# asharakeh/bayes-od-rc

Hardware: AMD Instinct MI355X
Metric: images/sec at N=10 MC samples, 512x512; per-anchor covariance latency (higher is better)
Workload: dtype bf16; 1 GPU; ResNet-50 RetinaNet + covar head, N=10 MC-dropout, 512x512, full BayesOD pipeline (forward+posterior+soft-NMS+cluster-fuse); global_batch=512, mc_samples=10, anchors=49104, parallelism=one GPU (no exchange; N > 1: image-sharded, one RCCL gather/step), visible_gpus=1, gpu_max_hw_queues=4

## Files before the change

### bayes-od-rc_amd/csrc/engine.hip

```cpp
#include "../../include/bayesod.h"
#include "kernels.h"
#include "jpeg_entropy.h"
#include "png_inflate.h"

#include <algorithm>
#include <array>
#include <atomic>
#include <chrono>
#include <cmath>
#include <condition_variable>
#include <deque>
#include <functional>
#include <mutex>
#include <thread>
#include <tuple>
#include <type_traits>
#include <cstdarg>
#include <cstdio>
#include <cstring>
#include <map>
#include <memory>
#include <string>
#include <system_error>
#include <vector>
#include <dlfcn.h>

namespace {

constexpr float BN_EPS = 1e-3f;

thread_local std::string g_create_error;

struct HostTensor { std::vector<int64_t> shape; std::vector<float> data; };

struct Plane {
    char* d = nullptr;
    int64_t base = 0;
    int64_t bstride = 0;
    int h = 0, w = 0, C = 0, pitch = 0;
};

struct PackedConv { char* w = nullptr; float* bias = nullptr; int cout = 0, cout_pad = 0, taps = 0, kw = 0, cin = 0; };

struct Op {
    enum Kind { STEM, POOL, CONV, KEEP } kind;
    ConvArgs conv;
    bool is_head3x3 = false;
    double flops = 0;
    std::string name;
    std::string wname[3], bnname[3];
    bool same_geom = false;
    int flavour = 0;
    int head[3] = {-1, -1, -1};
    bool hx_pyramid = false;
// ... 207 lines not shown
    int32_t* energy_list = nullptr; float* energy_term = nullptr;

    int sh = 0, sw = 0, ph = 0, pw = 0;
    int ch[6] = {0}, cw[6] = {0};
    int nlev = 0; int lh[8] = {0}, lw[8] = {0};
    int64_t lvl_off[8] = {0};
    int64_t lvl_p0[8] = {0};
    int64_t Ppad = 0; int P = 0, A = 0;

    std::map<std::string, HostTensor> host_w;
    std::map<std::string, PackedConv> packed;
    float* stem_w = nullptr; float* stem_b = nullptr;
    bool weights_ready = false, anchors_ready = false, forward_done = false, posterior_done = false,
         nms_done = false, cluster_done = false;

    float* d_images = nullptr;
    float* splitk_partial = nullptr; size_t splitk_elems = 0;
    uint8_t* d_frames_u8 = nullptr; size_t frames_u8_cap = 0;
    float* d_images_b[2] = {nullptr, nullptr}; uint8_t* d_u8_b[2] = {nullptr, nullptr}; size_t u8_cap_b[2] = {0, 0};
    hipStream_t copy = nullptr;
    hipEvent_t ev_img_ready[2] = {nullptr, nullptr}, ev_img_free[2] = {nullptr, nullptr};
    bool img_ready_pending[2] = {false, false}, img_free_pending[2] = {false, false};
    int cur_img_buf = -1;
    struct RaggedTable { std::vector<char> host; char* dev = nullptr; };
    RaggedTable rag_sync, rag_b[2];
    RaggedTable aug_sync, aug_b[2];
    JpegSlot jpeg_slot[3];
    PngSlot png_slot[3];
    CorruptSpec corrupt_pending;
    CorruptSlot corrupt_slot[3];
    hipEvent_t ev_tab[2] = {nullptr, nullptr};
    const float* kscale_src[2] = {nullptr, nullptr};
    float* kscale_cur[2] = {nullptr, nullptr}; int kscale_i = 0;
    const float* kscale_now = nullptr;
    char* stem_out = nullptr;
    int es = 2;
    bool split = false;
    char* pyr_hx = nullptr;
    int pyr_fmt = 1;
    int plan_mx = 0;
    int mx = 0;
    Plane pyramid;
    char* head_act[3][2] = {{nullptr}};
    char* head_act_t[3][4] = {{nullptr}};
    float* raw[3] = {nullptr};
    float* agg[3] = {nullptr};
    bool agg_plan = false;
    bool plan_fused_out = false, plan_xreuse = false, plan_xreuse0 = false;
    bool raw_valid = false, agg_valid = false;
    bool plan_sparse = false;
    bool plan_halo = false;
    SparseTailArgs sparse{};
    int plan_tail_rows = 0;
    bool agg_sparse = false;
    float* stat_acc[3] = {nullptr};
    int stat_k = 0;
    hipEvent_t ev_stat = nullptr;
    float* d_mirror = nullptr;
    int mirror_sym = -1, mirror_bad_level = 0;
    bool keep_ready = false;
    uint64_t keep_seed = 0; uint32_t keep_first = 0;
    uint64_t last_seed = 0; uint32_t last_first_image = 0;
    int32_t last_sample_base = 0;
    std::map<std::string, RowEnt*> tables;
    struct XrTable { RowEnt* rows = nullptr; int2* ext = nullptr; int m = 0; };
    std::map<std::string, XrTable> xr_tables;
    std::vector<Op> ops;
    const float* cur_images = nullptr;

    float* d_anchors = nullptr;
    PostBuffers pb{};
    float* nms_scores = nullptr; int32_t* nms_begin = nullptr;
    int32_t* nms_sel_s[2] = {nullptr, nullptr}; int32_t* nms_nsel_s[2] = {nullptr, nullptr};
    float* out_scores_s[2] = {nullptr, nullptr}; float* out_means_s[2] = {nullptr, nullptr};
    float* out_covs_s[2] = {nullptr, nullptr}; float* out_counts_s[2] = {nullptr, nullptr};
    int32_t* nms_sel = nullptr; int32_t* nms_nsel = nullptr;
    float* out_scores = nullptr; float* out_means = nullptr; float* out_covs = nullptr; float* out_counts = nullptr;
    int slot = 0;
    float* parts = nullptr;
    float* out_parts_s[2] = {nullptr, nullptr}; float* out_parts = nullptr;
    std::vector<char> parts_ok, det_parts_ok[2];
    bool parts_staged[2] = {false, false};
    bool class_parts = false;
    float* ent = nullptr; float* stat_ent = nullptr; int stat_ent_k = 0;
    float* cparts = nullptr;
    float* out_cparts_s[2] = {nullptr, nullptr}; float* out_cparts = nullptr;
    std::vector<char> cparts_ok, det_cparts_ok[2];
    bool cparts_staged[2] = {false, false};
    hipStream_t side = nullptr;
    int overlap_mode = 0;
    int ov_front_slots = 0, ov_slots = 0;
    hipStream_t full = nullptr, front = nullptr, back = nullptr;
    hipEvent_t ev_front_done[2] = {nullptr, nullptr}, ev_l0_done[2] = {nullptr, nullptr}, ev_join = nullptr;
    bool l0_pending[2] = {false, false};
    bool ov_dirty = false;
    char* pyr_d[2] = {nullptr, nullptr};
    int fwd_parity = 0, pyr_last = 0;
    int first_head_op = 0;
    bool in_overlap_call = false;
    int n_cu = 256;
    hipEvent_t ev_posterior = nullptr; hipEvent_t ev_done[2] = {nullptr, nullptr};
    int dev_op_lo = 0, dev_op_hi = 1 << 30;
    hipStream_t done_stream[2] = {nullptr, nullptr};
    bool side_pending[2] = {false, false};
    char* host_stage[2] = {nullptr, nullptr};
    float* rec_send = nullptr; float* rec_recv = nullptr; size_t rec_recv_elems = 0;
// ... 17 lines not shown
        va_list ap; va_start(ap, fmt); vsnprintf(buf, sizeof buf, fmt, ap); va_end(ap);
        err = buf;
        return s;
    }
    template <typename T> bod_status dalloc(T** p, size_t n_elems, bool zero = true) {
        void* q = nullptr;
        const size_t bytes = std::max<size_t>(n_elems * sizeof(T), 256);
        hipError_t e = hipMalloc(&q, bytes);
        if (e != hipSuccess) return fail(BOD_ERR_OOM, "hipMalloc(%zu) failed: %s", bytes, hipGetErrorString(e));
        if (zero) {
            e = hipMemsetAsync(q, 0, bytes, stream);
            if (e != hipSuccess) return fail(BOD_ERR_HIP, "hipMemset: %s", hipGetErrorString(e));
        }
        allocs.push_back(q);
        alloc_bytes[q] = bytes;
        device_bytes += (int64_t)bytes;
        *p = reinterpret_cast<T*>(q);
        return BOD_OK;
    }
};

#define HIPCHK(h, expr)                                                                         \
    do {                                                                                        \
        hipError_t _e = (expr);                                                                 \
        if (_e != hipSuccess)                                                                   \
            return (h)->fail(BOD_ERR_HIP, "%s failed: %s (%s:%d)", #expr, hipGetErrorString(_e), \
                             __FILE__, __LINE__);                                               \
    } while (0)
#define BODCHK(expr) do { bod_status _s = (expr); if (_s != BOD_OK) return _s; } while (0)

namespace {

const char* kHeadPrefix[3] = {"pyramid_classification", "pyramid_regression", "pyramid_cov"};
const int kHeadConvs[3] = {4, 3, 4};

void cu_slot_mask(int lo, int hi, uint32_t mask[8]) {
    for (int w = 0; w < 8; ++w) mask[w] = 0u;
    for (int slot = lo; slot < hi; ++slot)
        for (int xcd = 0; xcd < 8; ++xcd) { const int bit = slot * 8 + xcd; mask[bit >> 5] |= 1u << (bit & 31); }
}

int same_pad_before(int in, int k, int s) {
    const int out = (in + s - 1) / s;
    const int total = std::max((out - 1) * s + k - in, 0);
    return total / 2;
}

bod_status new_plane(bod_context* h, Plane* p, int B, int hh, int ww, int C) {
    p->h = hh; p->w = ww; p->C = C; p->pitch = ww + 2; p->base = 0;
    p->bstride = (int64_t)(hh + 2) * (ww + 2);
    return h->dalloc(&p->d, (size_t)B * p->bstride * C * h->es);
}

bod_status make_table(bod_context* h, const std::string& key, int B, const Plane& in, const Plane& out,
                      int stride, int org_y, int org_x, const Plane* res, const RowEnt** tbl) {
    auto it = h->tables.find(key);
    if (it != h->tables.end()) { *tbl = it->second; return BOD_OK; }
    std::vector<RowEnt> rows((size_t)B * out.h * out.w);
    size_t r = 0;
    for (int b = 0; b < B; ++b)
        for (int y = 0; y < out.h; ++y)
            for (int x = 0; x < out.w; ++x) {
                RowEnt e{};
                e.in_off = (int32_t)(in.base + b * in.bstride + (int64_t)(y * stride + org_y) * in.pitch + (x * stride + org_x));
                e.in_pitch = in.pitch;
                e.out_off = (int32_t)(out.base + b * out.bstride + (int64_t)(y + 1) * out.pitch + (x + 1));
                if (res) {
                    int ry = y, rx = x;
                    if (res->h != out.h || res->w != out.w) {
                        ry = std::min((int)std::floor((y + 0.5) * ((double)res->h / out.h)), res->h - 1);
                        rx = std::min((int)std::floor((x + 0.5) * ((double)res->w / out.w)), res->w - 1);
                    }
                    e.res_off = (int32_t)(res->base + b * res->bstride + (int64_t)(ry + 1) * res->pitch + (rx + 1));
                }
                rows[r++] = e;
            }
    RowEnt* d = nullptr;
    BODCHK(h->dalloc(&d, rows.size(), false));
    HIPCHK(h, hipMemcpyAsync(d, rows.data(), rows.size() * sizeof(RowEnt), hipMemcpyHostToDevice, h->stream));
    HIPCHK(h, hipStreamSynchronize(h->stream));
    h->tables[key] = d;
    *tbl = d;
    return BOD_OK;
}

const HostTensor* find_w(bod_context* h, const std::string& name, int kind) {
    auto it = h->host_w.find(name + "/" + std::to_string(kind));
    return it == h->host_w.end() ? nullptr : &it->second;
}

bod_status pack_conv(bod_context* h, const std::string& name, const std::string& bn, int cout_pad_to,
                     PackedConv* out, int hx = 0) {
    const std::string ckey = hx == 2 ? name + ":h4" : hx ? name + ":hx" : name;
    auto it = h->packed.find(ckey);
    if (it != h->packed.end()) { *out = it->second; return BOD_OK; }
    const HostTensor* k = find_w(h, name, 0);
    if (!k || k->shape.size() != 4) return h->fail(BOD_ERR_NOT_READY, "missing conv kernel '%s'", name.c_str());
    const int kh = (int)k->shape[0], kw = (int)k->shape[1], cin = (int)k->shape[2], cout = (int)k->shape[3];
    const HostTensor* b = find_w(h, name, 1);
    std::vector<double> scale(cout, 1.0), shift(cout, 0.0);
    for (int o = 0; o < cout; ++o) shift[o] = b ? (double)b->data[o] : 0.0;
    if (!bn.empty()) {
        const HostTensor *g = find_w(h, bn, 2), *be = find_w(h, bn, 3), *mu = find_w(h, bn, 4), *var = find_w(h, bn, 5);
        if (!g || !be || !mu || !var) return h->fail(BOD_ERR_NOT_READY, "missing batch-norm '%s'", bn.c_str());
        for (int o = 0; o < cout; ++o) {
            const double s = (double)g->data[o] / std::sqrt((double)var->data[o] + (double)BN_EPS);
            scale[o] = s;
            shift[o] = (shift[o] - (double)mu->data[o]) * s + (double)be->data[o];
        }
    }
    PackedConv pc;
    pc.cout = cout; pc.taps = kh * kw; pc.kw = kw; pc.cin = cin;
    pc.cout_pad = ((cout + cout_pad_to - 1) / cout_pad_to) * cout_pad_to;
    const size_t nw = (size_t)pc.cout_pad * pc.taps * cin;
    const bool as_f32 = h->es == 4 && !h->split;
    std::vector<uint16_t> w(as_f32 ? 0 : nw * (h->split ? 2 : 1), 0);
    std::vector<float> w32(as_f32 ? nw : 0, 0.f);
    std::vector<float> bias(pc.cout_pad, 0.f);
    for (int o = 0; o < cout; ++o) {
        bias[o] = (float)shift[o];
        for (int t = 0; t < pc.taps; ++t)
            for (int c = 0; c < cin; ++c) {
                const double v = (double)k->data[((size_t)t * cin + c) * cout + o] * scale[o];
                const size_t idx = ((size_t)o * pc.taps + t) * cin + c;
                if (h->split) {
                    const float f = (float)v;
                    const uint16_t hi = f2bf(f);
                    const size_t slot = ((size_t)o * pc.taps + t) * 2 * cin + (size_t)(c >> 5) * 64 + (c & 31);
                    w[slot] = hi; w[slot + 32] = f2bf(f - bf2f(hi));
// ... 5 lines not shown
        if (!h->split || cin % 64 != 0) return h->fail(BOD_ERR_INVALID_ARG, "hx weights need the (hi, lo) data path and cin %% 64 == 0");
        std::vector<float> row(cin);
        uint8_t* wb = reinterpret_cast<uint8_t*>(w.data());
        for (int o = 0; o < cout; ++o)
            for (int t = 0; t < pc.taps; ++t) {
                for (int c = 0; c < cin; ++c) row[c] = (float)((double)k->data[((size_t)t * cin + c) * cout + o] * scale[o]);
                if (hx == 2) {
                    if (cin != 256) return h->fail(BOD_ERR_INVALID_ARG, "h4 weights: 256 input channels");
                    pack_h4_row(row.data(), cin, wb + ((size_t)o * pc.taps + t) * cin * 4, true);
                } else pack_hx_row(row.data(), cin, wb + ((size_t)o * pc.taps + t) * cin * 4, true);
            }
    }
    size_t w_extra = 0;
    if (hx == 2) {
        if (pc.cout_pad != 256) return h->fail(BOD_ERR_INVALID_ARG, "h4 weights: one 256-cout tile");
        w_extra = (size_t)pc.taps * 2 * 2048;
        w.resize(w.size() + w_extra / 2, 0);
        uint8_t* wb = reinterpret_cast<uint8_t*>(w.data());
        uint8_t* sc = wb + nw * h->es;
        for (int t = 0; t < pc.taps; ++t)
            for (int x = 0; x < 2; ++x)
                for (int o = 0; o < 256; ++o)
                    std::memcpy(sc + ((size_t)(t * 2 + x) * 256 + o) * 8, wb + ((size_t)o * pc.taps + t) * cin * 4 + 768 + 8 * x, 8);
    }
    BODCHK(h->dalloc(&pc.w, nw * h->es + w_extra, false));
    BODCHK(h->dalloc(&pc.bias, bias.size(), false));
    HIPCHK(h, hipMemcpyAsync(pc.w, as_f32 ? (const void*)w32.data() : (const void*)w.data(), nw * h->es + w_extra,
                             hipMemcpyHostToDevice, h->stream));
    HIPCHK(h, hipMemcpyAsync(pc.bias, bias.data(), bias.size() * 4, hipMemcpyHostToDevice, h->stream));
    HIPCHK(h, hipStreamSynchronize(h->stream));
    h->packed[ckey] = pc;
    *out = pc;
    return BOD_OK;
}

ConvArgs base_args(const PackedConv& pc, const RowEnt* rows, int M, int in_cstride, int out_cstride) {
    ConvArgs a{};
    a.rows = rows; a.M = M; a.taps = pc.taps; a.KW = pc.kw; a.cin = pc.cin;
    a.in_cstride = in_cstride; a.cout_pad = pc.cout_pad; a.cout_valid = pc.cout;
    a.out_cstride = out_cstride; a.res_cstride = out_cstride; a.groups = 1;
    a.fan_count = 1; a.fan_stride = 0;
    return a;
}

void to_split_args(ConvArgs* a) {
    a->split = 1;
    a->cin *= 2; a->in_cstride *= 2; a->res_cstride *= 2;
    if (!(a->flags & CONV_OUT_F32)) a->out_cstride *= 2;
    for (int g = 0; g < 3; ++g) a->g[g].in_coff *= 2;
}

bod_status add_conv(bod_context* h, const std::string& name, const std::string& bn, const Plane& in,
                    const Plane& out, int stride, bool same, bool relu, const Plane* res,
                    char* out_relu = nullptr) {
    PackedConv pc;
    BODCHK(pack_conv(h, name, bn, 64, &pc));
    if (pc.cin != in.C || pc.cout != out.C)
        return h->fail(BOD_ERR_INVALID_ARG, "conv '%s': weight shape [%d->%d] does not match planes [%d->%d]",
                       name.c_str(), pc.cin, pc.cout, in.C, out.C);
    const int kh = pc.taps / pc.kw;
    int oy = 1, ox = 1;
    if (same) { oy = 1 - same_pad_before(in.h, kh, stride); ox = 1 - same_pad_before(in.w, pc.kw, stride); }
    char key[256];
    snprintf(key, sizeof key, "pp:%lld,%lld,%d:%lld,%lld,%d,%d,%d:%d:%d:%d:%lld,%lld,%d,%d,%d", (long long)in.base,
             (long long)in.bstride, in.pitch, (long long)out.base, (long long)out.bstride, out.pitch, out.h, out.w,
             stride, oy, ox, res ? (long long)res->base : -1LL, res ? (long long)res->bstride : 0LL,
             res ? res->pitch : 0, res ? res->h : 0, res ? res->w : 0);
    const RowEnt* tbl = nullptr;
    const int B = h->cfg.batch;
    BODCHK(make_table(h, key, B, in, out, stride, oy, ox, res, &tbl));
    Op op; op.kind = Op::CONV;
    op.conv = base_args(pc, tbl, B * out.h * out.w, in.C, out.C);
    op.conv.g[0] = ConvGroup{in.d, pc.w, pc.bias, out.d, res ? res->d : nullptr, out_relu, 0, 0, nullptr, nullptr, nullptr, 0, 0};
    op.conv.flags = relu ? CONV_RELU : 0;
    op.flops = 2.0 * op.conv.M * pc.cout * pc.taps * pc.cin;
    op.name = name; op.wname[0] = name; op.bnname[0] = bn;
    op.same_geom = stride == 1 && same && pc.taps == 9 && pc.kw == 3 && in.base == out.base && in.bstride == out.bstride && in.pitch == out.pitch &&
                   in.h == out.h && in.w == out.w;
    if (stride == 1 && same && pc.taps == 9 && pc.kw == 3 && in.h == out.h && in.w == out.w) { op.conv.plane_h = out.h; op.conv.plane_w = out.w; }
    static const bool splitk_on = [] { const char* e = getenv("BOD_CONV_SPLITK"); return !e || atoi(e) != 0; }();
    if (splitk_on && (h->es == 2 || h->split)) {
        const long tiles = (long)((op.conv.M + 127) / 128) * (pc.cout_pad % 128 == 0 ? pc.cout_pad / 128 : pc.cout_pad / 64);
        const int chunks = pc.cin * (h->split ? 2 : 1) / 64;
        int S = 1;
        while (tiles * S < 256 && S * 2 <= 16 && chunks % (S * 2) == 0 && (long)pc.taps * (chunks / (S * 2)) >= 4) S *= 2;
        if (S > 1) {
            op.conv.ksplit = S;
            h->splitk_elems = std::max(h->splitk_elems, (size_t)S * op.conv.M * pc.cout_pad);
        }
    }
    static const bool plane_xr_on = [] { const char* e = getenv("BOD_PLANE_XREUSE"); return !e || atoi(e) != 0; }();
    static const bool xr_on = [] { const char* e = getenv("BOD_CONV_XREUSE"); return !e || atoi(e) != 0; }();
    if (plane_xr_on && xr_on && (h->es == 2 || h->split) && !h->cfg.training && op.conv.ksplit <= 1 && stride == 1 && same && pc.taps == 9 && pc.kw == 3 &&
        pc.cin == 256 && pc.cout == 256 && pc.cout_pad == 256 && !res && !out_relu && in.h == out.h && in.w == out.w) {
        ConvArgs probe = op.conv;
        if (conv_igemm_uses_full_cout_tile(probe)) {
            const std::string xkey = std::string(key) + ":xr";
            auto it = h->xr_tables.find(xkey);
            if (it == h->xr_tables.end()) {
                std::vector<RowEnt> rows((size_t)op.conv.M), tiled;
                std::vector<ExtRow> ext;
                HIPCHK(h, hipMemcpy(rows.data(), tbl, rows.size() * sizeof(RowEnt), hipMemcpyDeviceToHost));
                if (!xr_tile_rows(rows, tiled, ext)) return h->fail(BOD_ERR_INVALID_ARG, "row-reuse tiling of '%s': extended rows out of order", name.c_str());
                bod_context::XrTable t;
                t.m = (int)tiled.size();
                BODCHK(h->dalloc(&t.rows, tiled.size(), false));
                BODCHK(h->dalloc(&t.ext, ext.size(), false));
                HIPCHK(h, hipMemcpy(t.rows, tiled.data(), tiled.size() * sizeof(RowEnt), hipMemcpyHostToDevice));
                HIPCHK(h, hipMemcpy(t.ext, ext.data(), ext.size() * sizeof(int2), hipMemcpyHostToDevice));
                it = h->xr_tables.emplace(xkey, t).first;
            }
            op.conv.rows = it->second.rows; op.conv.ext = it->second.ext; op.conv.M = it->second.m; op.conv.xreuse = 2;
        }
    }
    h->ops.push_back(op);
    return BOD_OK;
}

bod_status build_geometry(bod_context* h) {
    const bod_config& c = h->cfg;
    const int H = c.image_h, W = c.image_w;
    if (H < 64 || W < 64) return h->fail(BOD_ERR_INVALID_ARG, "image size %dx%d too small", H, W);
    h->sh = (H - 7) / 2 + 1; h->sw = (W - 7) / 2 + 1;
    h->ph = (h->sh + 2 - 3) / 2 + 1; h->pw = (h->sw + 4 - 3) / 2 + 1;
    h->ch[2] = h->ph; h->cw[2] = h->pw;
    for (int s = 3; s <= 5; ++s) { h->ch[s] = (h->ch[s - 1] - 1) / 2 + 1; h->cw[s] = (h->cw[s - 1] - 1) / 2 + 1; }
    if (c.min_level != 3 || c.max_level != 7)
        return h->fail(BOD_ERR_INVALID_ARG, "only pyramid levels 3..7 are supported (got %d..%d)", c.min_level, c.max_level);
    h->nlev = 5;
    h->lh[0] = h->ch[3]; h->lw[0] = h->cw[3];
    h->lh[1] = h->ch[4]; h->lw[1] = h->cw[4];
    h->lh[2] = h->ch[5]; h->lw[2] = h->cw[5];
    h->lh[3] = (h->lh[2] + 1) / 2; h->lw[3] = (h->lw[2] + 1) / 2;
    h->lh[4] = (h->lh[3] + 1) / 2; h->lw[4] = (h->lw[3] + 1) / 2;
    int64_t pp = 0; int p = 0;
    for (int l = 0; l < 5; ++l) {
        const int stride = 1 << (l + 3);
        const int ah = (H + stride - 1) / stride, aw = (W + stride - 1) / stride;
        if (ah != h->lh[l] || aw != h->lw[l])
            return h->fail(BOD_ERR_INVALID_ARG,
                           "pyramid level p%d is %dx%d but the anchor grid is %dx%d for a %dx%d image "
                           "(the reference's tf.concat of head outputs with anchors would mismatch too)",
                           l + 3, h->lh[l], h->lw[l], ah, aw, H, W);
        h->lvl_off[l] = pp; h->lvl_p0[l] = p;
        pp += (int64_t)(h->lh[l] + 2) * (h->lw[l] + 2);
        p += h->lh[l] * h->lw[l];
    }
    h->Ppad = pp; h->P = p; h->A = p * c.anchors_per_location;
    return BOD_OK;
}

Plane level_view(bod_context* h, int l) {
    Plane v = h->pyramid;
    v.base = h->lvl_off[l]; v.h = h->lh[l]; v.w = h->lw[l]; v.pitch = h->lw[l] + 2;
    return v;
}

bod_status ensure_raw(bod_context* h) {
    const bod_config& c = h->cfg;
    const int out_ch[3] = {c.anchors_per_location * c.num_classes, c.anchors_per_location * 4, c.anchors_per_location * 10};
    for (int hd = 0; hd < 3; ++hd) {
        if ((hd == 2 && !c.has_covar_head) || h->raw[hd]) continue;
        BODCHK(h->dalloc(&h->raw[hd], (size_t)c.batch * c.mc_samples * h->P * out_ch[hd]));
    }
    for (Op& o : h->ops)
// ... 4 lines not shown
}

bod_status train_init(bod_context* h);
bod_status train_forward_only(bod_context* h, const float* dev, uint64_t seed, uint32_t first_image_id);
const uint32_t* train_dyn_rng(bod_context* h);
void train_destroy(bod_context* h);
void val_destroy(bod_context* h);

bod_status ensure_stat(bod_context* h) {
    if (h->stat_acc[0]) return BOD_OK;
    const bod_config& c = h->cfg;
    const size_t BA = (size_t)c.batch * h->A;
    BODCHK(h->dalloc(&h->stat_acc[0], BA * c.num_classes));
    BODCHK(h->dalloc(&h->stat_acc[1], BA * 16));
    if (c.has_covar_head) BODCHK(h->dalloc(&h->stat_acc[2], BA * 10));
    if (c.covariance_parts & BOD_PARTS_CLASS) BODCHK(h->dalloc(&h->stat_ent, BA));
    return BOD_OK;
}

bod_status build_plan(bod_context* h) {
    const bod_config& c = h->cfg;
    const int B = c.batch, N = c.mc_samples;
    const bool train_mode = c.training != 0;
    h->ops.clear();
    {
        const HostTensor* k = find_w(h, "conv1", 0);
        if (!k || k->shape.size() != 4 || k->shape[0] != 7 || k->shape[2] != 3 || k->shape[3] != 64)
            return h->fail(BOD_ERR_NOT_READY, "missing / malformed stem kernel 'conv1' [7,7,3,64]");
        const HostTensor* b = find_w(h, "conv1", 1);
        const HostTensor *g = find_w(h, "bn_conv1", 2), *be = find_w(h, "bn_conv1", 3), *mu = find_w(h, "bn_conv1", 4), *var = find_w(h, "bn_conv1", 5);
        if (!g || !be || !mu || !var) return h->fail(BOD_ERR_NOT_READY, "missing batch-norm 'bn_conv1'");
        std::vector<float> w(7 * 7 * 3 * 64), bias(64);
        for (int o = 0; o < 64; ++o) {
            const double s = (double)g->data[o] / std::sqrt((double)var->data[o] + (double)BN_EPS);
            bias[o] = (float)((((b ? (double)b->data[o] : 0.0) - (double)mu->data[o]) * s) + (double)be->data[o]);
            for (int t = 0; t < 147; ++t) w[(size_t)t * 64 + o] = (float)((double)k->data[(size_t)t * 64 + o] * s);
        }
        BODCHK(h->dalloc(&h->stem_w, w.size(), false));
        BODCHK(h->dalloc(&h->stem_b, bias.size(), false));
        HIPCHK(h, hipMemcpyAsync(h->stem_w, w.data(), w.size() * 4, hipMemcpyHostToDevice, h->stream));
        HIPCHK(h, hipMemcpyAsync(h->stem_b, bias.data(), bias.size() * 4, hipMemcpyHostToDevice, h->stream));
        HIPCHK(h, hipStreamSynchronize(h->stream));
        BODCHK(h->dalloc(&h->stem_out, (size_t)B * h->sh * h->sw * 64 * h->es));
        Op s; s.kind = Op::STEM; s.name = "conv1(stem)"; s.flops = 2.0 * B * h->sh * h->sw * 64.0 * 147.0; h->ops.push_back(s);
        Op p; p.kind = Op::POOL; p.name = "pool1"; h->ops.push_back(p);
    }
    Plane x;
    BODCHK(new_plane(h, &x, B, h->ph, h->pw, 64));
    Plane pool_out = x;
    h->ops[1].conv.g[0].out = pool_out.d;
    const char* blocks[6] = {"", "", "abc", "abcd", c.backbone_depth == 101 ? "abcdefghijklmnopqrstuvw" : "abcdef", "abc"};
    const int f1s[6] = {0, 0, 64, 128, 256, 512};
    Plane taps[6];
    for (int st = 2; st <= 5; ++st) {
        const int f1 = f1s[st], f3 = f1 * 4, hh = h->ch[st], ww = h->cw[st];
        const int first_stride = st == 2 ? 1 : 2;
        Plane t1, t2, sc, oa, ob;
        BODCHK(new_plane(h, &t1, B, hh, ww, f1));
        BODCHK(new_plane(h, &t2, B, hh, ww, f1));
        BODCHK(new_plane(h, &sc, B, hh, ww, f3));
        BODCHK(new_plane(h, &oa, B, hh, ww, f3));
        BODCHK(new_plane(h, &ob, B, hh, ww, f3));
        bool use_a = true;
        int chain_stages = 0;
        if (const char* e = getenv("BOD_CHAIN_FUSION")) chain_stages = atoi(e);
        bool chain_ok = h->es == 2 && !h->split && !train_mode && ((st == 2 && chain_stages >= 1) || (st == 3 && chain_stages >= 3));
        Plane t1alt;
        if (chain_ok) BODCHK(new_plane(h, &t1alt, B, hh, ww, f1));
        bool t1_ready = false;
        bool pw_t1_ready = false;
        for (const char* bl = blocks[st]; *bl; ++bl) {
            char cb[64], bb[64];
            snprintf(cb, sizeof cb, "res%d%c_branch", st, *bl);
            snprintf(bb, sizeof bb, "bn%d%c_branch", st, *bl);
            const std::string c_(cb), b_(bb);
            if (chain_ok) {
                Plane& out = use_a ? oa : ob;
                const bool first = *bl == 'a';
                if (!t1_ready) BODCHK(add_conv(h, c_ + "2a", b_ + "2a", x, t1, first ? first_stride : 1, false, true, nullptr));
                if (first) BODCHK(add_conv(h, c_ + "1", b_ + "1", x, sc, first_stride, false, false, nullptr));
                BODCHK(add_conv(h, c_ + "2b", b_ + "2b", t1, t2, 1, true, true, nullptr));
                Op& op2b = h->ops.back();
                const Plane& shortcut = first ? sc : x;
                const bool can = op2b.conv.ksplit <= 1 && !conv_igemm_uses_big_tile(op2b.conv) && op2b.conv.cout_pad == f1 && (f1 == 64 || f1 == 128);
                if (!can) {
                    BODCHK(add_conv(h, c_ + "2c", b_ + "2c", t2, out, 1, false, true, &shortcut));
                    t1_ready = false;
                } else {
                    PackedConv p2c;
                    BODCHK(pack_conv(h, c_ + "2c", b_ + "2c", 64, &p2c));
                    if (p2c.cin != f1 || p2c.cout != f3 || p2c.taps != 1 || p2c.cout_pad != f3)
                        return h->fail(BOD_ERR_INVALID_ARG, "conv '%s2c' must be 1x1 %d->%d", cb, f1, f3);
                    ConvGroup& G = op2b.conv.g[0];
                    G.ch_w2 = p2c.w; G.ch_b2 = p2c.bias; G.ch_res = shortcut.d; G.ch_out = out.d; G.ch_c2 = f3;
                    op2b.flops += 2.0 * op2b.conv.M * (double)f3 * f1;
                    op2b.name += "+2c"; op2b.wname[1] = c_ + "2c"; op2b.bnname[1] = b_ + "2c";
                    t1_ready = false;
                    if (bl[1] != 0) {
                        char nb[64], nbb[64];
                        snprintf(nb, sizeof nb, "res%d%c_branch2a", st, bl[1]);
                        snprintf(nbb, sizeof nbb, "bn%d%c_branch2a", st, bl[1]);
                        PackedConv p2a;
                        BODCHK(pack_conv(h, nb, nbb, 64, &p2a));
                        if (p2a.cin != f3 || p2a.cout != f1 || p2a.taps != 1 || p2a.cout_pad != f1)
                            return h->fail(BOD_ERR_INVALID_ARG, "conv '%s' must be 1x1 %d->%d", nb, f3, f1);
                        G.ch_w3 = p2a.w; G.ch_b3 = p2a.bias; G.ch_out3 = t1alt.d;
// ... 26 lines not shown
                PackedConv p2a;
                BODCHK(pack_conv(h, nb, nbb, 64, &p2a));
                if (p2a.cin != f3 || p2a.cout != f1 || p2a.taps != 1 || p2a.cout_pad != (st == 2 ? 64 : 128)) return BOD_OK;
                ConvGroup& G = op2c.conv.g[0];
                G.ch_w3 = p2a.w; G.ch_b3 = p2a.bias; G.ch_out3 = t1.d;
                op2c.flops += 2.0 * op2c.conv.M * (double)f1 * f3;
                op2c.name += std::string("+") + nb; op2c.wname[2] = nb; op2c.bnname[2] = nbb;
                pw_t1_ready = true;
                return BOD_OK;
            };
            if (train_mode) {
                BODCHK(new_plane(h, &t1, B, hh, ww, f1));
                BODCHK(new_plane(h, &t2, B, hh, ww, f1));
                BODCHK(new_plane(h, &sc, B, hh, ww, f3));
                BODCHK(new_plane(h, &oa, B, hh, ww, f3));
                BODCHK(new_plane(h, &ob, B, hh, ww, f3));
            }
            Plane& out = use_a ? oa : ob;
            if (*bl == 'a') {
                bool dual = false;
                if (st == 2 && !train_mode && h->es == 2 && !h->split) {
                    BODCHK(add_conv(h, c_ + "1", b_ + "1", x, sc, first_stride, false, false, nullptr));
                    Op& op1 = h->ops.back();
                    PackedConv p2a;
                    BODCHK(pack_conv(h, c_ + "2a", b_ + "2a", 64, &p2a));
                    if (conv_pointwise_can_fuse_dual(op1.conv) && op1.conv.ksplit <= 1 && p2a.cin == 64 && p2a.cout == f1 && f1 == 64 &&
                        p2a.taps == 1 && p2a.cout_pad == 64) {
                        ConvGroup& G = op1.conv.g[0];
                        G.ch_w3 = p2a.w; G.ch_b3 = p2a.bias; G.ch_out3 = t1.d; G.ch_dual = 1;
                        op1.flops += 2.0 * op1.conv.M * (double)f1 * 64.0;
                        op1.name += std::string("+") + c_ + "2a"; op1.wname[2] = c_ + "2a"; op1.bnname[2] = b_ + "2a";
                        dual = true;
                    } else {
                        h->ops.pop_back();
                    }
                }
                if (!dual) BODCHK(add_conv(h, c_ + "2a", b_ + "2a", x, t1, first_stride, false, true, nullptr));
                BODCHK(add_conv(h, c_ + "2b", b_ + "2b", t1, t2, 1, true, true, nullptr));
                if (!dual) BODCHK(add_conv(h, c_ + "1", b_ + "1", x, sc, first_stride, false, false, nullptr));
                BODCHK(add_conv(h, c_ + "2c", b_ + "2c", t2, out, 1, false, true, &sc));
                BODCHK(fuse_next_2a(bl));
                if (st == 3 || st == 4) {
                    taps[st] = out;
                    Plane fresh;
                    BODCHK(new_plane(h, &fresh, B, hh, ww, f3));
                    x = out;
                    if (use_a) oa = fresh; else ob = fresh;
                    use_a = !use_a;
                    continue;
                }
            } else {
                if (!pw_t1_ready) BODCHK(add_conv(h, c_ + "2a", b_ + "2a", x, t1, 1, false, true, nullptr));
                pw_t1_ready = false;
                BODCHK(add_conv(h, c_ + "2b", b_ + "2b", t1, t2, 1, true, true, nullptr));
                BODCHK(add_conv(h, c_ + "2c", b_ + "2c", t2, out, 1, false, true, &x));
                BODCHK(fuse_next_2a(bl));
            }
            x = out;
            use_a = !use_a;
        }
    }
    const Plane c5 = x, c4 = taps[4], c3 = taps[3];

    h->pyramid.C = 256; h->pyramid.bstride = h->Ppad;
    BODCHK(h->dalloc(&h->pyramid.d, (size_t)B * h->Ppad * 256 * h->es));
    Plane c5r, m4, m3, p6relu;
    BODCHK(new_plane(h, &c5r, B, h->lh[2], h->lw[2], 256));
    BODCHK(new_plane(h, &m4, B, h->lh[1], h->lw[1], 256));
    BODCHK(new_plane(h, &m3, B, h->lh[0], h->lw[0], 256));
    char* p6relu_buf = nullptr;
    BODCHK(h->dalloc(&p6relu_buf, (size_t)B * h->Ppad * 256 * h->es));
    p6relu = h->pyramid; p6relu.d = p6relu_buf;
    BODCHK(add_conv(h, "C5_reduced", "", c5, c5r, 1, false, false, nullptr));
    BODCHK(add_conv(h, "P5", "", c5r, level_view(h, 2), 1, true, false, nullptr));
    BODCHK(add_conv(h, "P6", "", c5, level_view(h, 3), 2, true, false, nullptr, p6relu_buf));
    {
        Plane v = p6relu; v.base = h->lvl_off[3]; v.h = h->lh[3]; v.w = h->lw[3]; v.pitch = h->lw[3] + 2;
        BODCHK(add_conv(h, "P7", "", v, level_view(h, 4), 2, true, false, nullptr));
    }
    BODCHK(add_conv(h, "C4_reduced", "", c4, m4, 1, false, false, &c5r));
    BODCHK(add_conv(h, "P4", "", m4, level_view(h, 1), 1, true, false, nullptr));
    BODCHK(add_conv(h, "C3_reduced", "", c3, m3, 1, false, false, &m4));
    BODCHK(add_conv(h, "P3", "", m3, level_view(h, 0), 1, true, false, nullptr));

    const size_t act_elems = (size_t)B * N * h->Ppad * 256 * h->es;
    for (int hd = 0; hd < 3; ++hd) {
        if (hd == 2 && !c.has_covar_head) continue;
        if (train_mode) {
            for (int l = 0; l < kHeadConvs[hd]; ++l) BODCHK(h->dalloc(&h->head_act_t[hd][l], act_elems));
            continue;
        }
        BODCHK(h->dalloc(&h->head_act[hd][0], act_elems));
        BODCHK(h->dalloc(&h->head_act[hd][1], act_elems));
    }
    const int out_ch[3] = {c.anchors_per_location * c.num_classes, c.anchors_per_location * 4, c.anchors_per_location * 10};
    std::vector<RowEnt> t1, t2, t3;
    {
        PyramidGeometry pg = pyramid_geometry(h->lh, h->lw);
        if (pg.Ppad != h->Ppad || pg.P != h->P) return h->fail(BOD_ERR_INVALID_ARG, "pyramid geometry mismatch");
        head_row_tables(pg, B, N, t1, t2, t3);
    }
    RowEnt *d1 = nullptr, *d2 = nullptr, *d3 = nullptr;
    BODCHK(h->dalloc(&d1, t1.size(), false));
    BODCHK(h->dalloc(&d2, t2.size(), false));
    BODCHK(h->dalloc(&d3, t3.size(), false));
    HIPCHK(h, hipMemcpyAsync(d1, t1.data(), t1.size() * sizeof(RowEnt), hipMemcpyHostToDevice, h->stream));
    HIPCHK(h, hipMemcpyAsync(d2, t2.data(), t2.size() * sizeof(RowEnt), hipMemcpyHostToDevice, h->stream));
    HIPCHK(h, hipMemcpyAsync(d3, t3.data(), t3.size() * sizeof(RowEnt), hipMemcpyHostToDevice, h->stream));
// ... 3079 lines not shown
        HIPCHK(h, launch_pack_records_parts(h->nms_nsel_s[sidx], h->out_scores_s[sidx], h->out_means_s[sidx], h->out_covs_s[sidx],
                                            h->out_counts_s[sidx], h->out_parts_s[sidx], h->rec_send, B, K, C, st));
    else
        HIPCHK(h, launch_pack_records(h->nms_nsel_s[sidx], h->out_scores_s[sidx], h->out_means_s[sidx], h->out_covs_s[sidx],
                                      h->out_counts_s[sidx], h->rec_send, B, K, C, st));
    float* recv = nullptr;
    if (rank == root) {
        if (world == 1 && !nccl_comm) recv = h->rec_send;
        else {
            if (h->rec_recv_elems < block * world) {
                if (h->rec_recv && h->rec_recv != h->rec_send) hipFree(h->rec_recv);
                h->rec_recv = nullptr; h->rec_recv_elems = 0;
                if (hipMalloc(reinterpret_cast<void**>(&h->rec_recv), block * world * 4) != hipSuccess)
                    return h->fail(BOD_ERR_OOM, "bod_gather_detections: %zu bytes", block * world * 4);
                h->rec_recv_elems = block * world;
            }
            recv = h->rec_recv;
        }
    }
    if (nccl_comm) {
        if (!rccl().load()) return h->fail(BOD_ERR_NOT_READY, "bod_gather_detections: librccl.so (ncclGather) could not be opened");
        const int rc = rccl().gather(h->rec_send, recv, block,  7, root, nccl_comm, st);
        if (rc != 0) return h->fail(BOD_ERR_HIP, "ncclGather: %s", rccl().errstr ? rccl().errstr(rc) : "error");
    }
    if (!h->ev_gather) HIPCHK(h, hipEventCreateWithFlags(&h->ev_gather, hipEventDisableTiming));
    if (rank == root && gathered_host) {
        HIPCHK(h, hipMemcpyAsync(gathered_host, recv, block * world * 4, hipMemcpyDeviceToHost, st));
        HIPCHK(h, hipEventRecord(h->ev_gather, st)); h->gather_stream = st;
        HIPCHK(h, hipEventSynchronize(h->ev_gather));
    } else {
        HIPCHK(h, hipEventRecord(h->ev_gather, st)); h->gather_stream = st;
    }
    if (!(rank == root && gathered_host) && slot >= 0) {
        HIPCHK(h, hipEventRecord(h->ev_done[slot], st));
    }
    if (gathered_device) *gathered_device = recv;
    return BOD_OK;
}

bod_status bod_plan_info(bod_handle h, int32_t* info8) {
    if (!h || !info8) return BOD_ERR_INVALID_ARG;
    if (!h->weights_ready) return h->fail(BOD_ERR_NOT_READY, "bod_plan_info: the plan is built by bod_finalize_weights");
    for (int i = 0; i < 8; ++i) info8[i] = 0;
    info8[0] = h->agg_plan; info8[1] = h->plan_fused_out; info8[2] = h->plan_xreuse; info8[3] = h->plan_xreuse0;
    info8[4] = (int32_t)h->ops.size();
    for (const Op& o : h->ops) if (o.kind == Op::CONV && !o.is_head3x3 && o.conv.xreuse) ++info8[5];
    info8[6] = h->plan_mx;
    info8[7] = h->plan_sparse;
    return BOD_OK;
}

bod_status bod_plan_info_n(bod_handle h, int32_t* info, int32_t n) {
    if (!h || !info || n < 0) return BOD_ERR_INVALID_ARG;
    int32_t all[10];
    BODCHK(bod_plan_info(h, all));
    all[8] = h->plan_halo;
    all[9] = h->plan_tail_rows;
    for (int i = 0; i < n && i < 10; ++i) info[i] = all[i];
    return BOD_OK;
}

static bod_status stat_handle(bod_handle h, const char* who) {
    if (!h->cfg.mc_statistics) return h->fail(BOD_ERR_INVALID_ARG, "%s: the handle was not created with mc_statistics = 1", who);
    BODCHK(join_overlap(h));
    HIPCHK(h, hipSetDevice(h->cfg.device));
    return ensure_stat(h);
}

static bod_status stat_view_ready(bod_handle h, const char* who, int32_t view) {
    if (view != BOD_VIEW_IDENTITY && view != BOD_VIEW_HFLIP)
        return h->fail(BOD_ERR_INVALID_ARG, "%s: view must be BOD_VIEW_IDENTITY (0) or BOD_VIEW_HFLIP (1), got %d", who, view);
    if (view == BOD_VIEW_IDENTITY) return BOD_OK;
    if (!h->anchors_ready) return h->fail(BOD_ERR_NOT_READY, "%s: bod_set_anchors has not been called (a mirrored view maps every anchor to its partner)", who);
    const bod_config& c = h->cfg;
    const int K = c.anchors_per_location;
    if (h->mirror_sym < 0) {
        std::vector<float> an((size_t)h->A * 4);
        HIPCHK(h, hipMemcpyAsync(an.data(), h->d_anchors, an.size() * 4, hipMemcpyDeviceToHost, h->stream));
        HIPCHK(h, hipStreamSynchronize(h->stream));
        const float fw = (float)c.image_w;
        int bad = -1;
        for (int l = 0; l < h->nlev && bad < 0; ++l) {
            const size_t off = (size_t)h->lvl_p0[l] * K;
            const int W = h->lw[l];
            for (int y = 0; y < h->lh[l] && bad < 0; ++y)
                for (int x = 0; x < W && bad < 0; ++x)
                    for (int k = 0; k < K; ++k) {
                        const float* s = &an[(off + ((size_t)y * W + x) * K + k) * 4];
                        const float* p = &an[(off + ((size_t)y * W + (W - 1 - x)) * K + k) * 4];
                        const float want[4] = {s[0], fw - s[1], s[2], s[3]};
                        if (memcmp(p, want, 16) != 0) { bad = l; break; }
                    }
        }
        h->mirror_sym = bad < 0; h->mirror_bad_level = bad < 0 ? 0 : c.min_level + bad;
    }
    if (!h->mirror_sym)
        return h->fail(BOD_ERR_INVALID_ARG, "%s: the anchors of pyramid level %d are not mirror-symmetric about image_w / 2 for a %dx%d image "
                       "(BOD_VIEW_HFLIP needs image_w to be a multiple of 2^max_level = %d)", who, h->mirror_bad_level, c.image_h, c.image_w,
                       1 << c.max_level);
    return BOD_OK;
}

static bod_status stat_fold(bod_handle h, const char* who, const float* cls, const float* box, const float* cov, int kb, int32_t view = BOD_VIEW_IDENTITY) {
    if (kb < 1) return h->fail(BOD_ERR_INVALID_ARG, "%s: a record of %d samples", who, kb);
    if (h->stat_k > (1 << 24) - kb) return h->fail(BOD_ERR_INVALID_ARG, "%s: more than 2^24 samples in one accumulator", who);
    if (h->class_parts && h->stat_ent_k != h->stat_k)
        return h->fail(BOD_ERR_NOT_READY, "%s: ent_sum holds %d of the record's %d samples (bod_stat_merge_entropy / bod_stat_set_entropy has not followed)", who, h->stat_ent_k, h->stat_k);
    StatMergeArgs m{};
    m.BA = (int64_t)h->cfg.batch * h->A; m.C = h->cfg.num_classes; m.ka = h->stat_k; m.kb = kb;
    m.acc_cls = h->stat_acc[0]; m.acc_box = h->stat_acc[1]; m.acc_cov = h->stat_acc[2];
    m.src_cls = cls; m.src_box = box; m.src_cov = h->cfg.has_covar_head ? cov : nullptr;
// ... 261 lines not shown
```

### bayes-od-rc_amd/engine.py

```python
import ctypes as C

import numpy as np

from . import _lib
from ._lib import BodConfig, BodSizes, as_f32, fptr, iptr

_KINDS = {"kernel": 0, "bias": 1, "gamma": 2, "beta": 3, "mean": 4, "var": 5}
PRECISIONS = {"bf16": 0, "fp32": 1, "bf16x3": 2, "f16mx": 3, "f16mx4": 4}
VIEWS = {"identity": _lib.BOD_VIEW_IDENTITY, "hflip": _lib.BOD_VIEW_HFLIP}


def make_config(image_hw, batch=1, mc_samples=10, num_classes=8, anchors_per_location=9, device=0,
                dropout_rate=0.3, use_full_covar=True, bayes_od_config=None, nms_config=None,
                has_covar_head=True, dataset_name='bdd', orig_size=None, nms_variant='A',
                num_categorical_draws=30, layers=(3, 4, 5, 6, 7), precision='bf16', mc_sample_base=0,
                mc_ensemble_size=0, training=False, backbone_depth=50, pipeline_overlap=False, mc_statistics=False,
                covariance_parts=False, class_parts=False):
    bo = bayes_od_config or {'ranking_method': 'score', 'dirichlet_prior': {'type': 'non_informative'},
                             'gaussian_prior': {'type': 'isotropic', 'isotropic_variance': 100000.0}}
    nms = nms_config or {'max_output_size': 100, 'iou_threshold': 0.5, 'soft_nms_sigma': 0.5}
    cfg = BodConfig()
    cfg.device = int(device)
    cfg.image_h, cfg.image_w = int(image_hw[0]), int(image_hw[1])
    cfg.batch, cfg.mc_samples = int(batch), int(mc_samples)
# ... 646 lines not shown

    def stat_device_pointers(self):
        ptrs = (C.c_void_p * 3)()
        self._chk(self.lib.bod_stat_device(self.h, ptrs, None))
        return [ptrs[i] for i in range(3)]

    @property
    def stat_samples(self):
        k = C.c_int32(0)
        self._chk(self.lib.bod_stat_device(self.h, None, C.byref(k)))
        return int(k.value)

    def get_statistics(self):
        n = (self.B, self.A)
        cls = np.empty(n + (self.Ccls,), np.float32)
        box = np.empty(n + (16,), np.float32)
        cov = np.empty(n + (10,), np.float32) if self.cfg.has_covar_head else None
        k = C.c_int32(0)
        self._chk(self.lib.bod_stat_get(self.h, fptr(cls), fptr(box), fptr(cov), C.byref(k)))
        return cls, box, cov, int(k.value)

    def set_statistics(self, cls_sum, box_moments, cov_sum=None, samples=0):
        n = (self.B, self.A)
        arrs = []
        for a, w in ((cls_sum, self.Ccls), (box_moments, 16), (cov_sum, 10)):
            a = as_f32(a) if a is not None else None
            if a is not None and a.shape != n + (w,):
                raise ValueError("statistics array of shape %s, expected %s" % (a.shape, n + (w,)))
            arrs.append(a)
        self._chk(self.lib.bod_stat_set(self.h, fptr(arrs[0]), fptr(arrs[1]), fptr(arrs[2]), int(samples)))

    def stat_posterior(self, seed=0, first_image_id=0):
        self._chk(self.lib.bod_stat_posterior(self.h, seed, first_image_id))

    def bench_head_conv(self, layer=1, variant=0, iters=10):
        ms, fl = C.c_double(0), C.c_double(0)
        self._chk(self.lib.bod_bench_head_conv(self.h, layer, variant, iters, C.byref(ms), C.byref(fl)))
        return ms.value, fl.value

    def gather_detections(self, slot=-1, comm=None, world=1, rank=0, root=0, want_host=True):
        w = int(self.lib.bod_record_width(self.h))
        out = None
        dev = C.c_void_p(0)
        if rank == root and want_host:
            out = np.empty((world, self.B, self.K, w), np.float32)
        self._chk(self.lib.bod_gather_detections(self.h, int(slot), C.c_void_p(int(comm) if comm else 0), int(world), int(rank), int(root),
                                                 out.ctypes.data if out is not None else None,
                                                 C.byref(dev) if rank == root else None))
        if rank == root and not want_host:
            return int(dev.value or 0), (world, self.B, self.K, w)
        return out

    def plan_info(self):
        info = (C.c_int32 * 10)()
        self._chk(self.lib.bod_plan_info_n(self.h, info, 10))
        return {"aggregating": bool(info[0]), "fused_head_outputs": bool(info[1]), "row_reuse": bool(info[2]),
                "fan_out_row_reuse": bool(info[3]), "ops": int(info[4]), "plane_row_reuse_layers": int(info[5]), "tower_mx": bool(info[6]), "tower_mx_format": int(info[6]),
                "sparse_tail": bool(info[7]), "sparse_halo": bool(info[8]), "sparse_tail_rows": int(info[9])}

    @property
    def aggregating(self):
        return self.plan_info()["aggregating"]

    def profile_begin(self, which=None):
        if which is not None:
            self._chk(self.lib.bod_profile_select(self.h, int(which)))
        self._chk(self.lib.bod_profile_begin(self.h))

    def profile_end(self):
        hm, pm, fl = C.c_double(0), C.c_double(0), C.c_double(0)
        hl, pl = C.c_int64(0), C.c_int64(0)
        self._chk(self.lib.bod_profile_end(self.h, C.byref(hm), C.byref(hl), C.byref(fl), C.byref(pm), C.byref(pl)))
        return {"head_conv_ms": hm.value, "head_conv_launches": hl.value, "head_conv_flops": fl.value,
                "posterior_ms": pm.value, "posterior_launches": pl.value}


def pack_ragged(frames, batch=None):
    frames = list(frames)
    if batch is not None and len(frames) != int(batch):
        raise ValueError("expected %d frames, got %d" % (int(batch), len(frames)))
    if not frames:
        raise ValueError("no frames to pack")
    for i, f in enumerate(frames):
        if not isinstance(f, np.ndarray) or f.dtype != np.uint8 or f.ndim != 3 or f.shape[2] != 3 or f.shape[0] < 1 or f.shape[1] < 1:
            raise ValueError("frame %d: expected a uint8 array of shape (h, w, 3), got %s %s" %
                             (i, getattr(f, "dtype", type(f).__name__), getattr(f, "shape", "")))
    sizes = np.asarray([f.shape[:2] for f in frames], np.int32)
    buf = np.empty(3 * int(np.sum(sizes[:, 0].astype(np.int64) * sizes[:, 1])), np.uint8)
    off = 0
    for f in frames:
        buf[off:off + f.size] = f.reshape(-1)
        off += f.size
    return buf, sizes


AUGMENT_DTYPE = np.dtype([("flip", "<i4"), ("scale", "<f4"), ("off_y", "<f4"), ("off_x", "<f4"), ("gain", "<f4"), ("bias", "<f4")])
AUGMENT_IDENTITY = {"flip": 0, "scale": 1.0, "off_y": 0.5, "off_x": 0.5, "gain": 1.0, "bias": 0.0}
AUGMENT_DEFAULTS = {"flip_probability": 0.5, "scale_range": [0.8, 1.25], "random_placement": True, "gain_range": [0.8, 1.2],
                    "bias_range": [-20.0, 20.0], "min_visible": 0.25}


def augment_records(aug, batch=None):
    if isinstance(aug, np.ndarray):
        if aug.dtype != AUGMENT_DTYPE:
            raise ValueError("augmentation records must have dtype AUGMENT_DTYPE, got %s" % (aug.dtype,))
        rec = np.ascontiguousarray(aug).reshape(-1)
    else:
        rec = np.empty(len(aug), AUGMENT_DTYPE)
        for i, d in enumerate(aug):
            unknown = set(d) - set(AUGMENT_IDENTITY)
            if unknown:
# ... 503 lines not shown
```

Baseline: 2373 images/sec.

## Compute only strided-consumed pixels at backbone stage ends

At the last bottleneck block of stages 2-4, the 2c conv now runs over a step-2 row table, computing only the output pixels that the next stage's stride-2 entry reads. For stage 4, the 2b conv's row-reuse tiling is also restricted to even output rows. The step-2 tables are embedded in the unused second half of the dense row-table entries to avoid a separate allocation. This is meant to cut backbone conv FLOPs in inference. It depends on downstream consumers reading only even positions and on the row-entry layout trick.

```diff
diff --git a/bayes-od-rc_amd/csrc/engine.hip b/bayes-od-rc_amd/csrc/engine.hip
--- a/bayes-od-rc_amd/csrc/engine.hip
+++ b/bayes-od-rc_amd/csrc/engine.hip
@@ -1,5 +1,6 @@
 #include "../../include/bayesod.h"
 #include "kernels.h"
+#include "plane_tables.h"
 #include "jpeg_entropy.h"
 #include "png_inflate.h"
 
@@ -313,6 +314,7 @@
     bool plan_halo = false;
     SparseTailArgs sparse{};
     int plan_tail_rows = 0;
+    int plan_stage_end = 0;
     bool agg_sparse = false;
     float* stat_acc[3] = {nullptr};
     int stat_k = 0;
@@ -436,29 +438,29 @@
     return h->dalloc(&p->d, (size_t)B * p->bstride * C * h->es);
 }
 
-bod_status make_table(bod_context* h, const std::string& key, int B, const Plane& in, const Plane& out,
-                      int stride, int org_y, int org_x, const Plane* res, const RowEnt** tbl) {
+PlaneGeom plane_geom(const Plane& p) { return PlaneGeom{p.base, p.bstride, p.pitch, p.h, p.w}; }
+
+bod_status make_table(bod_context* h, const std::string& key, const std::string& dense_key, int B, const Plane& in, const Plane& out,
+                      int stride, int org_y, int org_x, const Plane* res, int out_step, const RowEnt** tbl, int* M) {
+    *M = B * plane_step_count(out.h, out_step) * plane_step_count(out.w, out_step);
     auto it = h->tables.find(key);
     if (it != h->tables.end()) { *tbl = it->second; return BOD_OK; }
-    std::vector<RowEnt> rows((size_t)B * out.h * out.w);
-    size_t r = 0;
-    for (int b = 0; b < B; ++b)
-        for (int y = 0; y < out.h; ++y)
-            for (int x = 0; x < out.w; ++x) {
-                RowEnt e{};
-                e.in_off = (int32_t)(in.base + b * in.bstride + (int64_t)(y * stride + org_y) * in.pitch + (x * stride + org_x));
-                e.in_pitch = in.pitch;
-                e.out_off = (int32_t)(out.base + b * out.bstride + (int64_t)(y + 1) * out.pitch + (x + 1));
-                if (res) {
-                    int ry = y, rx = x;
-                    if (res->h != out.h || res->w != out.w) {
-                        ry = std::min((int)std::floor((y + 0.5) * ((double)res->h / out.h)), res->h - 1);
-                        rx = std::min((int)std::floor((x + 0.5) * ((double)res->w / out.w)), res->w - 1);
-                    }
-                    e.res_off = (int32_t)(res->base + b * res->bstride + (int64_t)(ry + 1) * res->pitch + (rx + 1));
-                }
-                rows[r++] = e;
-            }
+    std::vector<RowEnt> rows;
+    const PlaneGeom gi = plane_geom(in), go = plane_geom(out), gr = res ? plane_geom(*res) : PlaneGeom{};
+    plane_row_table(B, gi, go, stride, org_y, org_x, res ? &gr : nullptr, out_step, rows);
+    if (out_step != 1) {
+        const RowEnt* dense = nullptr;
+        int Md = 0;
+        BODCHK(make_table(h, dense_key, dense_key, B, in, out, stride, org_y, org_x, res, 1, &dense, &Md));
+        RowEnt* view = const_cast<RowEnt*>(dense);
+        if (rows.size() < (size_t)Md) {
+            view = const_cast<RowEnt*>(plane_step_view(dense));
+            HIPCHK(h, hipMemcpy2D(view, sizeof(RowEnt), rows.data(), sizeof(RowEnt), PLANE_STEP_VIEW_BYTES, rows.size(), hipMemcpyHostToDevice));
+        }
+        h->tables[key] = view;
+        *tbl = view;
+        return BOD_OK;
+    }
     RowEnt* d = nullptr;
     BODCHK(h->dalloc(&d, rows.size(), false));
     HIPCHK(h, hipMemcpyAsync(d, rows.data(), rows.size() * sizeof(RowEnt), hipMemcpyHostToDevice, h->stream));
@@ -570,7 +572,7 @@
 
 bod_status add_conv(bod_context* h, const std::string& name, const std::string& bn, const Plane& in,
                     const Plane& out, int stride, bool same, bool relu, const Plane* res,
-                    char* out_relu = nullptr) {
+                    char* out_relu = nullptr, int out_step = 1, bool even_rows = false) {
     PackedConv pc;
     BODCHK(pack_conv(h, name, bn, 64, &pc));
     if (pc.cin != in.C || pc.cout != out.C)
@@ -579,16 +581,18 @@
     const int kh = pc.taps / pc.kw;
     int oy = 1, ox = 1;
     if (same) { oy = 1 - same_pad_before(in.h, kh, stride); ox = 1 - same_pad_before(in.w, pc.kw, stride); }
-    char key[256];
-    snprintf(key, sizeof key, "pp:%lld,%lld,%d:%lld,%lld,%d,%d,%d:%d:%d:%d:%lld,%lld,%d,%d,%d", (long long)in.base,
-             (long long)in.bstride, in.pitch, (long long)out.base, (long long)out.bstride, out.pitch, out.h, out.w,
-             stride, oy, ox, res ? (long long)res->base : -1LL, res ? (long long)res->bstride : 0LL,
-             res ? res->pitch : 0, res ? res->h : 0, res ? res->w : 0);
+    char key[256], dense_key[256];
+    for (int k = 0; k < 2; ++k)
+        snprintf(k ? dense_key : key, sizeof key, "pp:%lld,%lld,%d:%lld,%lld,%d,%d,%d:%d:%d:%d:%lld,%lld,%d,%d,%d:%d", (long long)in.base,
+                 (long long)in.bstride, in.pitch, (long long)out.base, (long long)out.bstride, out.pitch, out.h, out.w,
+                 stride, oy, ox, res ? (long long)res->base : -1LL, res ? (long long)res->bstride : 0LL,
+                 res ? res->pitch : 0, res ? res->h : 0, res ? res->w : 0, k ? 1 : out_step);
     const RowEnt* tbl = nullptr;
     const int B = h->cfg.batch;
-    BODCHK(make_table(h, key, B, in, out, stride, oy, ox, res, &tbl));
+    int M = 0;
+    BODCHK(make_table(h, key, dense_key, B, in, out, stride, oy, ox, res, out_step, &tbl, &M));
     Op op; op.kind = Op::CONV;
-    op.conv = base_args(pc, tbl, B * out.h * out.w, in.C, out.C);
+    op.conv = base_args(pc, tbl, M, in.C, out.C);
     op.conv.g[0] = ConvGroup{in.d, pc.w, pc.bias, out.d, res ? res->d : nullptr, out_relu, 0, 0, nullptr, nullptr, nullptr, 0, 0};
     op.conv.flags = relu ? CONV_RELU : 0;
     op.flops = 2.0 * op.conv.M * pc.cout * pc.taps * pc.cin;
@@ -598,7 +602,7 @@
     if (stride == 1 && same && pc.taps == 9 && pc.kw == 3 && in.h == out.h && in.w == out.w) { op.conv.plane_h = out.h; op.conv.plane_w = out.w; }
     static const bool splitk_on = [] { const char* e = getenv("BOD_CONV_SPLITK"); return !e || atoi(e) != 0; }();
     if (splitk_on && (h->es == 2 || h->split)) {
-        const long tiles = (long)((op.conv.M + 127) / 128) * (pc.cout_pad % 128 == 0 ? pc.cout_pad / 128 : pc.cout_pad / 64);
+        const long tiles = (long)((B * out.h * out.w + 127) / 128) * (pc.cout_pad % 128 == 0 ? pc.cout_pad / 128 : pc.cout_pad / 64);
         const int chunks = pc.cin * (h->split ? 2 : 1) / 64;
         int S = 1;
         while (tiles * S < 256 && S * 2 <= 16 && chunks % (S * 2) == 0 && (long)pc.taps * (chunks / (S * 2)) >= 4) S *= 2;
@@ -613,12 +617,15 @@
         pc.cin == 256 && pc.cout == 256 && pc.cout_pad == 256 && !res && !out_relu && in.h == out.h && in.w == out.w) {
         ConvArgs probe = op.conv;
         if (conv_igemm_uses_full_cout_tile(probe)) {
-            const std::string xkey = std::string(key) + ":xr";
+            bool even = even_rows;
+            if (even) { ConvArgs half = op.conv; half.M = B * plane_step_count(out.h, 2) * out.w; even = conv_igemm_uses_full_cout_tile(half); }
+            const std::string xkey = std::string(key) + (even ? ":xr:even" : ":xr");
             auto it = h->xr_tables.find(xkey);
             if (it == h->xr_tables.end()) {
                 std::vector<RowEnt> rows((size_t)op.conv.M), tiled;
                 std::vector<ExtRow> ext;
                 HIPCHK(h, hipMemcpy(rows.data(), tbl, rows.size() * sizeof(RowEnt), hipMemcpyDeviceToHost));
+                if (even) { std::vector<RowEnt> dense; dense.swap(rows); plane_rows_of_even_y(dense, B, out.h, out.w, rows); }
                 if (!xr_tile_rows(rows, tiled, ext)) return h->fail(BOD_ERR_INVALID_ARG, "row-reuse tiling of '%s': extended rows out of order", name.c_str());
                 bod_context::XrTable t;
                 t.m = (int)tiled.size();
@@ -629,6 +636,7 @@
                 it = h->xr_tables.emplace(xkey, t).first;
             }
             op.conv.rows = it->second.rows; op.conv.ext = it->second.ext; op.conv.M = it->second.m; op.conv.xreuse = 2;
+            if (even) op.flops = 2.0 * B * plane_step_count(out.h, 2) * out.w * pc.cout * pc.taps * pc.cin;
         }
     }
     h->ops.push_back(op);
@@ -739,6 +747,9 @@
     const char* blocks[6] = {"", "", "abc", "abcd", c.backbone_depth == 101 ? "abcdefghijklmnopqrstuvw" : "abcdef", "abc"};
     const int f1s[6] = {0, 0, 64, 128, 256, 512};
     Plane taps[6];
+    int stage_end = train_mode ? 0 : 2;
+    if (const char* e = getenv("BOD_STAGE_END_PIXELS")) stage_end = std::min(stage_end, std::max(atoi(e), 0));
+    h->plan_stage_end = stage_end;
     for (int st = 2; st <= 5; ++st) {
         const int f1 = f1s[st], f3 = f1 * 4, hh = h->ch[st], ww = h->cw[st];
         const int first_stride = st == 2 ? 1 : 2;
@@ -871,8 +882,9 @@
             } else {
                 if (!pw_t1_ready) BODCHK(add_conv(h, c_ + "2a", b_ + "2a", x, t1, 1, false, true, nullptr));
                 pw_t1_ready = false;
-                BODCHK(add_conv(h, c_ + "2b", b_ + "2b", t1, t2, 1, true, true, nullptr));
-                BODCHK(add_conv(h, c_ + "2c", b_ + "2c", t2, out, 1, false, true, &x));
+                const bool stage_end_blk = bl[1] == 0 && st <= 4;
+                BODCHK(add_conv(h, c_ + "2b", b_ + "2b", t1, t2, 1, true, true, nullptr, nullptr, 1, stage_end_blk && stage_end >= 2 && st == 4));
+                BODCHK(add_conv(h, c_ + "2c", b_ + "2c", t2, out, 1, false, true, &x, nullptr, stage_end_blk && stage_end >= 1 ? 2 : 1));
                 BODCHK(fuse_next_2a(bl));
             }
             x = out;
@@ -4058,11 +4070,12 @@
 
 bod_status bod_plan_info_n(bod_handle h, int32_t* info, int32_t n) {
     if (!h || !info || n < 0) return BOD_ERR_INVALID_ARG;
-    int32_t all[10];
+    int32_t all[11];
     BODCHK(bod_plan_info(h, all));
     all[8] = h->plan_halo;
     all[9] = h->plan_tail_rows;
-    for (int i = 0; i < n && i < 10; ++i) info[i] = all[i];
+    all[10] = h->plan_stage_end;
+    for (int i = 0; i < n && i < 11; ++i) info[i] = all[i];
     return BOD_OK;
 }
 
diff --git a/bayes-od-rc_amd/csrc/plane_tables.h b/bayes-od-rc_amd/csrc/plane_tables.h
--- /dev/null
+++ b/bayes-od-rc_amd/csrc/plane_tables.h
@@ -0,0 +1,61 @@
+#pragma once
+#include "plan_tables.h"
+#include <cmath>
+
+struct PlaneGeom {
+    int64_t base;
+    int64_t bstride;
+    int pitch;
+    int h, w;
+};
+
+inline int plane_step_count(int n, int step) { return (n + step - 1) / step; }
+
+inline RowEnt plane_row_entry(const PlaneGeom& in, const PlaneGeom& out, int stride, int org_y, int org_x, const PlaneGeom* res, int b, int y, int x) {
+    RowEnt e{};
+    e.in_off = (int32_t)(in.base + b * in.bstride + (int64_t)(y * stride + org_y) * in.pitch + (x * stride + org_x));
+    e.in_pitch = in.pitch;
+    e.out_off = (int32_t)(out.base + b * out.bstride + (int64_t)(y + 1) * out.pitch + (x + 1));
+    if (res) {
+        int ry = y, rx = x;
+        if (res->h != out.h || res->w != out.w) {
+            ry = std::min((int)std::floor((y + 0.5) * ((double)res->h / out.h)), res->h - 1);
+            rx = std::min((int)std::floor((x + 0.5) * ((double)res->w / out.w)), res->w - 1);
+        }
+        e.res_off = (int32_t)(res->base + b * res->bstride + (int64_t)(ry + 1) * res->pitch + (rx + 1));
+    }
+    return e;
+}
+
+inline void plane_row_table(int B, const PlaneGeom& in, const PlaneGeom& out, int stride, int org_y, int org_x, const PlaneGeom* res,
+                            int out_step, std::vector<RowEnt>& rows) {
+    const int ny = plane_step_count(out.h, out_step), nx = plane_step_count(out.w, out_step);
+    rows.resize((size_t)B * ny * nx);
+    size_t r = 0;
+    for (int b = 0; b < B; ++b)
+        for (int y = 0; y < ny; ++y)
+            for (int x = 0; x < nx; ++x) rows[r++] = plane_row_entry(in, out, stride, org_y, org_x, res, b, y * out_step, x * out_step);
+}
+
+constexpr size_t PLANE_STEP_VIEW_BYTES = 16;
+static_assert(sizeof(RowEnt) == 32 && offsetof(RowEnt, rng_p) == PLANE_STEP_VIEW_BYTES, "the step-2 view starts at an entry's second half");
+
+inline bool plane_embed_step_table(std::vector<RowEnt>& dense, const std::vector<RowEnt>& step) {
+    if (step.size() >= dense.size()) return false;
+    for (size_t i = 0; i < step.size(); ++i) {
+        dense[i].rng_p = step[i].in_off; dense[i].rng_zs = step[i].in_pitch; dense[i].pad0 = step[i].out_off; dense[i].pad1 = step[i].res_off;
+    }
+    return true;
+}
+
+inline const RowEnt* plane_step_view(const RowEnt* dense) {
+    return reinterpret_cast<const RowEnt*>(reinterpret_cast<const char*>(dense) + PLANE_STEP_VIEW_BYTES);
+}
+
+inline void plane_rows_of_even_y(const std::vector<RowEnt>& dense, int B, int h, int w, std::vector<RowEnt>& rows) {
+    rows.clear();
+    rows.reserve((size_t)B * plane_step_count(h, 2) * w);
+    for (int b = 0; b < B; ++b)
+        for (int y = 0; y < h; y += 2)
+            for (int x = 0; x < w; ++x) rows.push_back(dense[((size_t)b * h + y) * w + x]);
+}
diff --git a/bayes-od-rc_amd/engine.py b/bayes-od-rc_amd/engine.py
--- a/bayes-od-rc_amd/engine.py
+++ b/bayes-od-rc_amd/engine.py
@@ -722,11 +722,12 @@
         return out
 
     def plan_info(self):
-        info = (C.c_int32 * 10)()
-        self._chk(self.lib.bod_plan_info_n(self.h, info, 10))
+        info = (C.c_int32 * 11)()
+        self._chk(self.lib.bod_plan_info_n(self.h, info, 11))
         return {"aggregating": bool(info[0]), "fused_head_outputs": bool(info[1]), "row_reuse": bool(info[2]),
                 "fan_out_row_reuse": bool(info[3]), "ops": int(info[4]), "plane_row_reuse_layers": int(info[5]), "tower_mx": bool(info[6]), "tower_mx_format": int(info[6]),
-                "sparse_tail": bool(info[7]), "sparse_halo": bool(info[8]), "sparse_tail_rows": int(info[9])}
+                "sparse_tail": bool(info[7]), "sparse_halo": bool(info[8]), "sparse_tail_rows": int(info[9]),
+                "stage_end_pixels": int(info[10])}
 
     @property
     def aggregating(self):
```

New measurement: 2405 images/sec (median of 6 runs). 1.01x the previous value.
